# Lynx-MR/orbslam3lib

Measured on AMD Instinct MI355X. Metric: Mfeatures/s extract + Mmatches/s BFMatch, 640x480 stereo 8-level pyr, 1/2/4/8 GPU, higher is better.
Workload: dtype u8; 1 GPU; C2 640x480 stereo, 8 levels x1.2, 2000 feat/frame, FAST 20/7, + per-pair 2000x2000 Hamming kNN2 (left->right, all rows); parallelism=frames sharded across 1 GPU(s), replicas

## Files before the change

### include/orbgpu.h

```cpp
#ifndef ORBGPU_H_
#define ORBGPU_H_

#include <stddef.h>
#include <stdint.h>

#ifdef __cplusplus
extern "C" {
#endif

#define ORBGPU_ABI_VERSION 2

enum {
    ORBGPU_OK = 0,
    ORBGPU_ERR_EMPTY_IMAGE = -1,
    ORBGPU_ERR_CAPACITY = -2,
    ORBGPU_ERR_INVALID = -3,
    ORBGPU_ERR_HIP = -4,
    ORBGPU_ERR_OVERFLOW = -5,
    ORBGPU_ERR_NO_DEVICE = -6,
    ORBGPU_ERR_RUNTIME = -7
};

typedef struct {
    int32_t nfeatures;
// ... 31 lines not shown

int orbgpu_upload_images(orbgpu_ctx* ctx, const uint8_t* images, int n_images, int width,
                         int height, int stride);
uint8_t* orbgpu_device_input(orbgpu_ctx* ctx);
int orbgpu_upload_images_async(orbgpu_ctx* ctx, const uint8_t* images, int n_images, int width,
                               int height, int stride);
int orbgpu_host_alloc(size_t bytes, void** ptr);
int orbgpu_host_free(void* ptr);
int orbgpu_run_batch(orbgpu_ctx* ctx, int n_images, int width, int height, const int32_t* laps,
                     void* stream);
int orbgpu_download_result(orbgpu_ctx* ctx, int image, orbgpu_keypoint* kps, uint8_t* desc,
                           int cap, int* n, int* n_mono);
int orbgpu_download_counts(orbgpu_ctx* ctx, int n_images, int32_t* n, int32_t* n_mono);
int orbgpu_candidate_counts(orbgpu_ctx* ctx, int n_images, int32_t* counts);
int orbgpu_synchronize(orbgpu_ctx* ctx);

int orbgpu_get_pyramid_level(orbgpu_ctx* ctx, int image, int level, int blurred, uint8_t* dst,
                             int dst_stride, int* width, int* height);

int orbgpu_get_level_keypoints(orbgpu_ctx* ctx, int image, orbgpu_keypoint* kps, uint8_t* desc,
                               int cap, int32_t* counts);

int orbgpu_match_knn2(orbgpu_ctx* ctx, const uint8_t* query, int nq, const uint8_t* train, int nt,
                      int32_t* idx1, int32_t* dist1, int32_t* idx2, int32_t* dist2);
int orbgpu_export_descriptors(orbgpu_ctx* ctx, int image, int row0, uint8_t* device_dst, int cap_rows,
                              int* n_rows, void* stream);
int orbgpu_match_knn2_device(orbgpu_ctx* ctx, const uint8_t* d_query, int nq, const uint8_t* d_train, int nt,
                             int32_t* d_idx1, int32_t* d_dist1, int32_t* d_idx2, int32_t* d_dist2, void* stream);

int orbgpu_ingest_images(orbgpu_ctx* ctx, const uint8_t* device_images, int n_images, int width,
// ... 129 lines not shown
```

### orbslam3lib_amd/__init__.py

```python
from __future__ import annotations

import ctypes as C
import os

import numpy as np

__all__ = ["ORBextractor", "ORBmatcher", "BFMatcher", "BatchExtractor", "KEYPOINT_DTYPE", "MAP_POINT_DTYPE",
           "LAST_POINT_DTYPE", "TRACK_POSE_DTYPE", "OrbGpuError", "load_library", "LIB_PATH"]

HERE = os.path.dirname(os.path.abspath(__file__))
LIB_PATH = os.environ.get("ORBGPU_LIB") or os.path.join(HERE, "liborbgpu.so")

MAP_POINT_DTYPE = np.dtype([("proj_x", "<f4"), ("proj_y", "<f4"), ("proj_xr", "<f4"), ("view_cos", "<f4"),
                            ("depth", "<f4"), ("level", "<i4"), ("flags", "<i4"), ("desc", "u1", (32,)),
                            ("proj_yr", "<f4"), ("view_cos_r", "<f4"), ("level_r", "<i4")])
MP_IN_VIEW, MP_BAD, MP_HAS_OBS, MP_IN_VIEW_R = 1, 2, 4, 8

LAST_POINT_DTYPE = np.dtype([("pos", "<f4", (3,)), ("angle", "<f4"), ("octave", "<i4"), ("flags", "<i4"),
                             ("desc", "u1", (32,))])
TRACK_POSE_DTYPE = np.dtype([("Rcw", "<f4", (9,)), ("tcw", "<f4", (3,)), ("Rlw", "<f4", (9,)), ("tlw", "<f4", (3,))])
LP_VALID = 1
TRACK_RIG_DTYPE = np.dtype([("cam_left", "<f4", (8,)), ("Rrl", "<f4", (9,)), ("trl", "<f4", (3,))])

KEYPOINT_DTYPE = np.dtype([("x", "<f4"), ("y", "<f4"), ("size", "<f4"), ("angle", "<f4"),
# ... 5 lines not shown
    "orbgpu_download_result", "orbgpu_download_counts", "orbgpu_synchronize",
    "orbgpu_get_pyramid_level", "orbgpu_get_level_keypoints", "orbgpu_match_knn2",
    "orbgpu_match_stereo_batch", "orbgpu_download_matches", "orbgpu_descriptor_distance",
    "orbgpu_stereo_matches_batch", "orbgpu_download_stereo", "orbgpu_candidate_counts",
    "orbgpu_image_bounds", "orbgpu_undistort_grid_batch", "orbgpu_download_grid",
    "orbgpu_device_sbs_input", "orbgpu_upload_sbs", "orbgpu_ingest_sbs", "orbgpu_pack_soa",
    "orbgpu_download_soa", "orbgpu_download_matches16", "orbgpu_extract_features",
    "orbgpu_search_by_projection_batch", "orbgpu_search_by_projection_stereo",
    "orbgpu_download_projection_matches", "orbgpu_upload_images_async", "orbgpu_host_alloc",
    "orbgpu_host_free", "orbgpu_export_descriptors", "orbgpu_match_knn2_device",
    "orbgpu_set_profiling", "orbgpu_num_stages", "orbgpu_stage_name", "orbgpu_stage_times",
    "orbgpu_reset_stage_times", "orbgpu_last_error", "orbgpu_abi_version",
    "orbgpu_fisheye_stereo_batch", "orbgpu_download_fisheye", "orbgpu_run_batch_match",
    "orbgpu_diagnostic_knobs", "orbgpu_ingest_images", "orbgpu_export_batch_bytes", "orbgpu_export_batch",
    "orbgpu_get_device", "orbgpu_track_by_projection_batch", "orbgpu_download_track_matches",
    "orbgpu_track_by_projection_stereo",
]

DEVICE_CURRENT = -1


class KB8Rig(C.Structure):
    _fields_ = [("cam_left", C.c_float * 8), ("cam_right", C.c_float * 8), ("precision_left", C.c_float),
                ("precision_right", C.c_float), ("R12", C.c_float * 9), ("t12", C.c_float * 3)]

    @classmethod
    def make(cls, cam_left, cam_right, R12=None, t12=(0.0, 0.0, 0.0), precision_left=1e-6,
             precision_right=1e-6):
        r = cls()
        r.cam_left[:] = [float(v) for v in cam_left]
        r.cam_right[:] = [float(v) for v in cam_right]
# ... 395 lines not shown
                                           C.c_void_p(stream) if stream else None))

    def match_stereo(self, stereo_rows_only=False, stream=None):
        _check(_lib.orbgpu_match_stereo_batch(self.ctx.handle, self.n // 2, int(stereo_rows_only),
                                              C.c_void_p(stream) if stream else None))

    def synchronize(self):
        _check(_lib.orbgpu_synchronize(self.ctx.handle))

    def counts(self):
        n = np.zeros(self.n, np.int32)
        m = np.zeros(self.n, np.int32)
        _check(_lib.orbgpu_download_counts(self.ctx.handle, self.n, _p(n), _p(m)))
        return n, m

    def candidate_counts(self):
        c = np.zeros(self.n, np.int32)
        _check(_lib.orbgpu_candidate_counts(self.ctx.handle, self.n, _p(c)))
        return c

    def result(self, i, cap=65536):
        kps = np.zeros(cap, KEYPOINT_DTYPE)
        desc = np.zeros((cap, 32), np.uint8)
        n, m = C.c_int(0), C.c_int(0)
        _check(_lib.orbgpu_download_result(self.ctx.handle, i, _p(kps), _p(desc), cap, C.byref(n),
                                           C.byref(m)))
        return kps[:n.value], desc[:n.value], m.value

    def matches(self, pair, cap=65536):
        out = [np.zeros(cap, np.int32) for _ in range(4)]
# ... 220 lines not shown
```

### orbslam3lib_amd/csrc/orb_ctx.h

```cpp
#pragma once
#include <hip/hip_runtime.h>

#include <algorithm>
#include <cstring>
#include <mutex>
#include <string>
#include <vector>

#include "../../include/orbgpu.h"
#include "orb_geometry.h"
#include "orb_kernels.h"

namespace orbgpu {

int fail(int code, const std::string& msg);

#define HIP_TRY(expr)                                                                  \
    do {                                                                               \
        hipError_t e_ = (expr);                                                        \
        if (e_ != hipSuccess)                                                          \
            return fail(ORBGPU_ERR_HIP, std::string(#expr) + ": " + hipGetErrorString(e_)); \
    } while (0)

enum Stage { ST_RESIZE, ST_BLUR, ST_FAST48, ST_FAST, ST_FAST_TOP, ST_OCTREE, ST_ORIENT, ST_FINAL, ST_KNN,
// ... 90 lines not shown
    int stereo_pairs = 0;
    int fisheye_pairs = 0;
    hipEvent_t fork = nullptr;
    hipEvent_t ext_done = nullptr;
    DevBuf input2{bufs};
    int in_slot = 0, pending_slot = -1;
    hipStream_t copy = nullptr;
    hipEvent_t slot_ready = nullptr;
    std::vector<hipEvent_t> slot_free;
    std::vector<hipEvent_t> join;
    bool serialize = false;
    struct GraphRec { int key[7]; hipGraphExec_t exec; unsigned long long used; };
    std::vector<GraphRec> graphs;
    unsigned long long graph_tick = 0;
    bool last_fused = false;
    std::vector<int32_t> laps_host;
    bool need_fork = true;
    bool restagger = false;
    std::vector<hipEvent_t> stagger_ev;
    std::vector<orbgpu::Chunk> last_chunks;
    int last_images = 0, last_w = 0, last_h = 0, last_pairs = 0;
    unsigned prof_mask = 0;
    std::vector<orbgpu::Pending> pending;
    std::vector<hipEvent_t> event_pool;
    double stage_ms[orbgpu::ST_COUNT] = {};
    long long stage_n[orbgpu::ST_COUNT] = {};
};

namespace orbgpu {

// ... 116 lines not shown
```

### orbslam3lib_amd/csrc/orb_geometry.h

```cpp
#pragma once
#include <algorithm>
#include <cfloat>
#include <climits>
#include <cmath>
#include <cstdlib>
#include <string>
#include <vector>

#include "../../include/orbgpu.h"
#include "orb_fast_cell.h"
#include "orb_kernels.h"
#include "orb_octree.h"

namespace orbgpu {

inline int round_up(int x, int a) { return (x + a - 1) / a * a; }
inline long long round_up_ll(long long x, long long a) { return (x + a - 1) / a * a; }
inline int cv_round_f(float v) { return (int)std::lrintf(v); }
inline int cv_round_d(double v) { return (int)std::lrint(v); }
inline int cv_floor_f(float v) { return (int)std::floor(v); }
inline short sat_short(float v) {
    int i = cv_round_f(v);
    return (short)std::min(std::max(i, (int)SHRT_MIN), (int)SHRT_MAX);
}
// ... 267 lines not shown
        A.oct_split_min_images = 0;
    } else {
        A.oct_split = layout(0) ? 0 : L;
        A.oct_split_min_images = kOctSmallMinImages;
    }
    A.oct_may_retry = 0;
    for (int l = 0; l < L; ++l) {
        const LevelGeom& G = A.lv[l];
        if (G.oct_cap > lds_nodes || G.ncells > A.oct_nq_off / 4) A.oct_may_retry = 1;
        if (l >= A.oct_split && (G.oct_cap > A.oct2_lds_nodes || G.ncells > A.oct2_nq_off / 4)) A.oct_may_retry = 1;
    }
    A.oct_force_retry = K.oct_generic ? 1 : 0;
    A.oct_pyr_max = K.oct_pyr_max;
    A.oct_rounds = K.oct_rounds ? 1 : 0;
    if (A.oct_force_retry) A.oct_may_retry = 1;
}

inline void fast_records(const GeomKnobs& K, GeomPlan& P) {
    BatchArgs& A = P.A;
    const int L = A.nlevels;
    auto fits = [&](int l, int pitch) { return A.lv[l].wCell + 9 <= pitch && A.lv[l].hCell + 6 <= pitch; };
    int tier[kMaxLevels];
    for (int l = 0; l < L; ++l) {
        const int t = fits(l, kCellPitchTiny) ? 0 : fits(l, kCellPitchSmall) ? 1 : 2;
        tier[l] = std::max(t, K.fast_min_tier);
    }
    A.fast_tab_off = (int)P.rtab.size();
    int tier_end[3] = {0, 0, 0}, nrec = 0;
    for (int t = 0; t < 3; ++t) {
        for (int l = 0; l < L; ++l) {
// ... 78 lines not shown
```

### orbslam3lib_amd/csrc/orb_kernels.h

```cpp
#pragma once
#include <hip/hip_runtime.h>
#include <stddef.h>
#include <stdint.h>

namespace orbgpu {

constexpr int kMaxLevels = 16;
constexpr int kMinBorder = 16;
constexpr int kEdge = 19;

__device__ inline int xcd_remap(int orig, int nwg) {
    const int xcd = orig % 8, q = nwg / 8, r = nwg % 8;
    return (xcd < r ? xcd * (q + 1) : r * (q + 1) + (xcd - r) * q) + orig / 8;
}

struct LevelGeom {
    int w, h, pitch;
    long long img_stride;
    int bpitch;
    long long bimg_stride;
    int nCols, nRows, wCell, hCell, maxBX, maxBY;
    int ncells, cell_cap;
    int cell_first;
    long long cellkey_off;
// ... 50 lines not shown
    int* fast_ovf_cnt;
    int fast_qcap;
    int fast_small, fast_ovf_all;
    unsigned long long* octdbg;
    int oct_lds_nodes;
    int oct_lds_bytes;
    int oct_nq_off;
    int oct_split;
    int oct_split_min_images;
    int oct2_threads;
    int oct2_lds_nodes, oct2_lds_bytes, oct2_nq_off, oct2_lds_keys;
    int oct_may_retry;
    int oct_force_retry;
    int oct_pyr_max;
    int oct_rounds;
    int tail0;
    int tail_lds, tail_buf1, tail_tab, tail_maxq, tail_maxrows;
    int tail_min;
    int fuse_out;
};

struct MatchArgs {
    const uint8_t* desc;
    const int32_t* out_n;
    const int32_t* out_mono;
    int out_cap;
    int stereo_only;
    int32_t* idx1;
    int32_t* dist1;
    int32_t* idx2;
// ... 68 lines not shown
    int32_t* cell_start;
    int32_t* cell_idx;
    int img0;
};

constexpr int kOctLdsNodes = 1024;
constexpr int kOdKpBlock = 8;
constexpr int kOdBlockKps = 3 * kOdKpBlock;

constexpr int kOctLdsKeys = 16384;
constexpr int kFastMergeMaxImages = 4;
template <int CP>
constexpr int kFastSmallList() { return CP == 48 ? 512 : 1280; }
constexpr int kFastOvfBlocks = 32;
constexpr int kOctSmallThreads = 256;
constexpr int kOctSmallMinImages = 32;
constexpr int kOctSmallLds = 51 * 1024;

struct OctCfg {
    int nq_off;
    int lds_nodes;
    int lds_keys;
    int lds_bytes;
};

struct OctLayout {
    long long keys, nq, nodemem, total;
};

__host__ __device__ inline long long oct_align(long long x) { return (x + 255) & ~255LL; }
// ... 176 lines not shown
```

### orbslam3lib_amd/csrc/orb_kernels.hip

```cpp
#include <hip/hip_runtime.h>
#include <stdint.h>

#include <algorithm>
#include <atomic>

#include "orb_kernels.h"
#include "orb_math.h"
#include "orb_fast_cell.h"
#include "orb_octree.h"
#include "orb_pattern_data.h"
#include "orb_policy.h"

namespace orbgpu {

static_assert(sizeof(BatchArgs) <= 4096, "kernel argument block too large");

struct PatternTable {
    int8_t v[1024];
};
constexpr int hexval(char c) { return c <= '9' ? c - '0' : c - 'a' + 10; }
constexpr PatternTable make_pattern() {
    PatternTable t{};
    const char* h = ORBGPU_PATTERN_HEX;
    for (int i = 0; i < 1024; ++i) t.v[i] = (int8_t)(hexval(h[2 * i]) * 16 + hexval(h[2 * i + 1]));
// ... 700 lines not shown
    if (nq == 0) return;
    for (int q = blockIdx.x; q < nq; q += gridDim.x) {
        const int2 e = a.fast_ovf[(long long)a.img0 * a.fast_qcap + q];
        fast_cell_one<CP, kList>(a, e.x, e.y, T, M, list, lut, emask, wcnt, wovf, scratch);
        __syncthreads();
    }
    if (threadIdx.x == 0) {
        const int done = __hip_atomic_fetch_add(cnt + 1, 1, __ATOMIC_RELAXED, __HIP_MEMORY_SCOPE_AGENT);
        if (done == (int)gridDim.x - 1) {
            __hip_atomic_store(cnt, 0, __ATOMIC_RELAXED, __HIP_MEMORY_SCOPE_AGENT);
            __hip_atomic_store(cnt + 1, 0, __ATOMIC_RELAXED, __HIP_MEMORY_SCOPE_AGENT);
        }
    }
}

constexpr int kOctRetry = -7;

template <bool kLdsPath>
__device__ __attribute__((always_inline)) inline void octree_level(const BatchArgs& a, int img, int l,
                                                                   uint8_t* nodemem_lds, int* scratch,
                                                                   OctShared& sh, const OctCfg q) {
    const LevelGeom G = a.lv[l];
    DevPolicy p{scratch};
    const int32_t* cnt = a.cellcnt + (long long)img * a.cellcnt_img_stride + G.cellcnt_off;
    const uint32_t* ck = a.cellkeys + (long long)img * a.cellkeys_img_stride + G.cellkey_off;
    uint8_t* ws = a.octws + (long long)img * a.octws_img_stride + G.oct_off;
    const OctLayout L = oct_layout(G.cand_cap, G.oct_cap);
    uint32_t* keys = reinterpret_cast<uint32_t*>(ws + L.keys);
    void* nm = G.oct_cap <= q.lds_nodes ? (void*)nodemem_lds : (void*)(ws + L.nodemem);
    int32_t* cell_off = reinterpret_cast<int32_t*>(nodemem_lds);
    const bool off_in_lds = G.ncells <= q.nq_off / 4;
    if (!off_in_lds) cell_off = reinterpret_cast<int32_t*>(ws + L.nq);
    auto scan_cells = [&]() {
        int carry = 0;
        for (int base = 0; base < G.ncells; base += blockDim.x) {
            const int i = base + threadIdx.x;
            const int v = i < G.ncells ? cnt[i] : 0;
            int tot;
            const int ex = p.scan_excl(v, &tot);
            if (i < G.ncells) cell_off[i] = carry + ex;
            carry += tot;
        }
        __syncthreads();
        return carry;
    };
    const int n = scan_cells();
    uint32_t* out_keys = a.lvlkey + (long long)img * a.lvlkp_img_stride + G.kp_off;
    unsigned long long* dbg = a.octdbg ? a.octdbg + ((long long)img * kMaxLevels + l) * 8 : nullptr;
    int r = n > G.cand_cap ? -3 : 0;
    const bool nodes_fit = off_in_lds && G.oct_cap <= q.lds_nodes && !a.oct_force_retry;
    const int pyr_off = (int)((max(oct_nodemem_bytes(G.oct_cap), (size_t)(4 * G.ncells)) + 15) & ~(size_t)15);
    const int pyrD = kLdsPath && q.lds_bytes > pyr_off && (long long)G.ncells * G.cell_cap < (1 << 24)
                         ? oct_pyr_depth((size_t)(q.lds_bytes - pyr_off), G.W, G.H, a.oct_pyr_max)
                         : 0;
    uint16_t* xtbl = reinterpret_cast<uint16_t*>(nodemem_lds + pyr_off + oct_pyr_bytes(pyrD, oct_nini(G.W, G.H)));
    if (kLdsPath && r == 0 && !nodes_fit) r = kOctRetry;
    if (kLdsPath && r == 0 && n > q.lds_keys) {
        OctWST<kLdsAS, kGlobalAS, kGlobalAS> w;
        w.keys = (asp<kGlobalAS, uint32_t>)keys;
        w.n = n;
        w.nq = (asp<kGlobalAS, uint16_t>)(ws + L.nq);
        w.m = oct_nodemem_carve<kLdsAS>(nodemem_lds, G.oct_cap);
        w.cap = G.oct_cap;
        w.out_keys = (asp<kGlobalAS, uint32_t>)out_keys;
        w.out_cap = G.kp_cap;
        w.dbg = dbg;
        w.cell_off = (asp<kLdsAS, const int32_t>)cell_off;
        w.cellkeys = (asp<kGlobalAS, const uint32_t>)ck;
        w.ncells = G.ncells;
        w.cell_cap = G.cell_cap;
        w.pyr = (asp<kLdsAS, uint32_t>)(nodemem_lds + pyr_off);
        w.pyrD = pyrD;
        w.rounds = a.oct_rounds;
        w.xcode = (asp<kLdsAS, uint16_t>)xtbl;
        w.ycode = (asp<kLdsAS, uint16_t>)(xtbl + G.W + 1);
        r = octree_distribute(p, w, (asp<kLdsAS, OctShared>)&sh, G.W, G.H, G.N);
        if (r == kOctDeep) {
            __syncthreads();
            scan_cells();
            w.pyrD = 0;
            r = octree_distribute(p, w, (asp<kLdsAS, OctShared>)&sh, G.W, G.H, G.N);
        }
    } else if (kLdsPath && r == 0) {
        OctWST<kLdsAS, kGlobalAS> w;
        w.keys = (asp<kGlobalAS, uint32_t>)keys;
        w.n = n;
        w.nq = (asp<kLdsAS, uint16_t>)(nodemem_lds + q.nq_off);
        w.m = oct_nodemem_carve<kLdsAS>(nodemem_lds, G.oct_cap);
        w.cap = G.oct_cap;
        w.out_keys = (asp<kGlobalAS, uint32_t>)out_keys;
        w.out_cap = G.kp_cap;
        w.dbg = dbg;
        w.cell_off = (asp<kLdsAS, const int32_t>)cell_off;
        w.cellkeys = (asp<kGlobalAS, const uint32_t>)ck;
        w.ncells = G.ncells;
        w.cell_cap = G.cell_cap;
        w.pyr = (asp<kLdsAS, uint32_t>)(nodemem_lds + pyr_off);
        w.pyrD = pyrD;
        w.rounds = a.oct_rounds;
        w.xcode = (asp<kLdsAS, uint16_t>)xtbl;
        w.ycode = (asp<kLdsAS, uint16_t>)(xtbl + G.W + 1);
        r = octree_distribute(p, w, (asp<kLdsAS, OctShared>)&sh, G.W, G.H, G.N);
        if (r == kOctDeep) {
            __syncthreads();
            scan_cells();
            w.pyrD = 0;
            r = octree_distribute(p, w, (asp<kLdsAS, OctShared>)&sh, G.W, G.H, G.N);
        }
    } else if (!kLdsPath && r == 0) {
        OctWST<kGeneric, kGeneric> w;
        w.keys = keys;
        w.n = n;
        w.nq = n <= q.lds_keys && off_in_lds ? reinterpret_cast<uint16_t*>(nodemem_lds + q.nq_off)
                                             : reinterpret_cast<uint16_t*>(ws + L.nq);
        w.m = oct_nodemem_carve<kGeneric>(nm, G.oct_cap);
        w.cap = G.oct_cap;
        w.out_keys = out_keys;
        w.out_cap = G.kp_cap;
        w.dbg = dbg;
        w.cell_off = cell_off;
        w.cellkeys = ck;
        w.ncells = G.ncells;
        w.cell_cap = G.cell_cap;
// ... 4 lines not shown
        else r = octree_distribute(p, w, &sh, G.W, G.H, G.N);
    }
    if (threadIdx.x == 0) {
        a.lvlcnt[img * kMaxLevels + l] = r < 0 ? 0 : r;
        a.status[img * kMaxLevels + l] = r < 0 ? r : 0;
    }
}

template <int NT>
__global__ __launch_bounds__(NT) void k_octree(BatchArgs a, int l0, OctCfg q) {
    extern __shared__ __attribute__((aligned(16))) uint8_t nodemem_lds[];
    __shared__ int scratch[16];
    __shared__ OctShared sh;
    octree_level<true>(a, a.img0 + blockIdx.x, l0 + blockIdx.y, nodemem_lds, scratch, sh, q);
}

__global__ __launch_bounds__(512, 1) void k_octree_retry(BatchArgs a) {
    extern __shared__ __attribute__((aligned(16))) uint8_t nodemem_lds[];
    __shared__ int scratch[16];
    __shared__ OctShared sh;
    for (int s = blockIdx.x; s < a.nimages * a.nlevels; s += gridDim.x) {
        const int img = a.img0 + s / a.nlevels, l = s % a.nlevels;
        if (a.status[img * kMaxLevels + l] != kOctRetry) continue;
        octree_level<false>(a, img, l, nodemem_lds, scratch, sh, OctCfg{a.oct_nq_off, a.oct_lds_nodes, kOctLdsKeys, a.oct_lds_bytes});
        __syncthreads();
    }
}

constexpr int kOdLanes = 32;
constexpr int kOdPairs = 256 / kOdLanes;
static_assert(kOdLanes == 32, "k_orient_desc: one disc row and 8 test pairs per lane");
static_assert(kOdKpBlock == 256 / kOdLanes, "orb_kernels.h kOdKpBlock");

constexpr int kOdPatchR = 18;
constexpr int kOdPatchRows = 2 * kOdPatchR + 1;
constexpr int kOdPatchPitch = 48;
constexpr int kOdPatchChunks = kOdPatchRows * 3;
constexpr int kOdPatchIt = (kOdPatchChunks + kOdLanes - 1) / kOdLanes;

__device__ inline int od_sum(int v) {
// ... 616 lines not shown
        hipLaunchKernelGGL((k_fast_cells<kCellPitchSmall, true>), grid, block, 0, s, a, c0, magic);
        hipLaunchKernelGGL(k_fast_cells_ovf<kCellPitchSmall>, dim3(kFastOvfBlocks), oblock, 0, s, a);
    } else if (tile == kCellPitchTiny) hipLaunchKernelGGL((k_fast_cells<kCellPitchTiny, false>), grid, block, 0, s, a, c0, magic);
    else if (tile == kCellPitchSmall) hipLaunchKernelGGL((k_fast_cells<kCellPitchSmall, false>), grid, block, 0, s, a, c0, magic);
    else hipLaunchKernelGGL((k_fast_cells<kCellMax, false>), grid, block, 0, s, a, c0, magic);
    return hipGetLastError();
}
hipError_t launch_octree(const BatchArgs& a, hipStream_t s) {
    constexpr int kMaxDevices = 64;
    static std::atomic<int> lds_set[kMaxDevices];
    int dev = 0;
    if (hipGetDevice(&dev) != hipSuccess || dev < 0 || dev >= kMaxDevices) dev = kMaxDevices - 1;
    std::atomic<int>& set = lds_set[dev];
    if (a.oct_lds_bytes > 65536 && a.oct_lds_bytes > set.load()) {
        for (const void* f : {reinterpret_cast<const void*>(k_octree<512>),
                              reinterpret_cast<const void*>(k_octree_retry)}) {
            hipError_t e = hipFuncSetAttribute(f, hipFuncAttributeMaxDynamicSharedMemorySize, a.oct_lds_bytes);
            if (e != hipSuccess) return e;
        }
        int cur = set.load();
        while (a.oct_lds_bytes > cur && !set.compare_exchange_weak(cur, a.oct_lds_bytes)) {}
    }
    const int split = a.nimages < a.oct_split_min_images ? a.nlevels : std::min(a.oct_split, a.nlevels);
    if (split > 0)
        hipLaunchKernelGGL(k_octree<512>, dim3(a.nimages, split), dim3(512), a.oct_lds_bytes, s, a, 0,
                           OctCfg{a.oct_nq_off, a.oct_lds_nodes, kOctLdsKeys, a.oct_lds_bytes});
    if (split < a.nlevels) {
        const OctCfg q{a.oct2_nq_off, a.oct2_lds_nodes, a.oct2_lds_keys, a.oct2_lds_bytes};
        if (a.oct2_threads == 128)
            hipLaunchKernelGGL(k_octree<128>, dim3(a.nimages, a.nlevels - split), dim3(128), a.oct2_lds_bytes, s, a,
                               split, q);
        else
            hipLaunchKernelGGL(k_octree<256>, dim3(a.nimages, a.nlevels - split), dim3(256), a.oct2_lds_bytes, s, a,
                               split, q);
    }
    if (a.oct_may_retry)
        hipLaunchKernelGGL(k_octree_retry, dim3(std::min(a.nimages * a.nlevels, 64)), dim3(512),
                           a.oct_lds_bytes, s, a);
    return hipGetLastError();
}
hipError_t launch_orient_desc(const BatchArgs& a, hipStream_t s) {
    const uint32_t d = (uint32_t)a.total_od_blocks;
    const uint32_t magic = d > 1 ? 0xFFFFFFFFu / d + 1u : 0u;
    hipLaunchKernelGGL(k_orient_desc, dim3(a.total_od_blocks, a.nimages), dim3(256), 0, s, a, magic);
    return hipGetLastError();
}
hipError_t launch_finalize(const BatchArgs& a, hipStream_t s) {
    if (a.nimages <= 2) hipLaunchKernelGGL(k_finalize<1024>, dim3(a.nimages), dim3(1024), 0, s, a);
    else if (a.nimages <= kFinWideMaxImages) hipLaunchKernelGGL(k_finalize<512>, dim3(a.nimages), dim3(512), 0, s, a);
    else hipLaunchKernelGGL(k_finalize<256>, dim3(a.nimages), dim3(256), 0, s, a);
    return hipGetLastError();
}
hipError_t launch_knn2_pairs(const MatchArgs& m, int npairs, hipStream_t s) {
// ... 24 lines not shown
```

### orbslam3lib_amd/csrc/orb_octree.h

```cpp
#pragma once
#include <hip/hip_runtime.h>
#include <stdint.h>

#include "orb_addrspace.h"
#include "orb_kernels.h"
#include "orb_introsort.h"

namespace orbgpu {

struct alignas(16) OctNode {
    uint16_t x0, y0, x1, y1;
    int32_t cnt;
    uint32_t path;
};
static_assert(sizeof(OctNode) == 16, "OctNode: 16 bytes");

constexpr int kOctPyrMaxD = 7;
constexpr int kOctDeep = -8;
__host__ __device__ inline int pyr_base(int d, int nIni) { return nIni * (((1 << (2 * d)) - 1) / 3); }
__host__ __device__ inline size_t oct_pyr_bytes(int D, int nIni) { return 8 * (size_t)pyr_base(D + 1, nIni); }
__host__ __device__ inline uint32_t oct_path_code(int d, uint32_t idx) { return ((uint32_t)d << 27) | idx; }
__host__ __device__ inline int oct_path_depth(uint32_t code) { return (int)(code >> 27); }
__host__ __device__ inline uint32_t oct_path_idx(uint32_t code) { return code & 0x7FFFFFFu; }
__host__ __device__ inline int oct_nini(int W, int H) {
    const int nIni = (int)roundf((float)W / (float)H);
    return nIni < 1 ? 1 : nIni;
}
__host__ __device__ inline size_t oct_tbl_bytes(int W, int H) { return ((size_t)2 * (W + H + 2) + 15) & ~(size_t)15; }
__host__ __device__ inline int oct_pyr_depth(size_t bytes, int W, int H, int Dmax) {
    const int nIni = oct_nini(W, H);
    const size_t t = oct_tbl_bytes(W, H);
    int D = 0;
    while (D < Dmax && D < kOctPyrMaxD && oct_pyr_bytes(D + 1, nIni) + t <= bytes &&
// ... 150 lines not shown
    n.y1 = (uint16_t)(v.y >> 16);
    n.cnt = (int32_t)v.z;
    n.path = v.w;
    return n;
}
template <class NP>
__host__ __device__ inline void on_st(NP a, int i, OctNode n) {
    orb_u32x4 v;
    v.x = (uint32_t)n.x0 | ((uint32_t)n.y0 << 16);
    v.y = (uint32_t)n.x1 | ((uint32_t)n.y1 << 16);
    v.z = (uint32_t)n.cnt;
    v.w = n.path;
    as_vec4(a)[i] = v;
}

template <int LAS, int GAS, int NAS, class P>
__host__ __device__ __attribute__((always_inline)) inline int octree_distribute(P& p, const OctWST<LAS, GAS, NAS> ws,
                                          asp<LAS, OctShared> sh, int W, int H, int N) {
    const int tid = p.tid(), NT = p.nthreads();
    const int n = ws.n;
    const OctNodeMemT<LAS> M = ws.m;
    auto cur = M.nodesA;
    auto nxt = M.nodesB;
    auto ccur = M.cntA;
    auto cnxt = M.cntB;
    auto vsz = M.vsizeA;
    auto vsz2 = M.vsizeB;
    auto nq = ws.nq;
    const bool nw = p.node_worker();
    unsigned long long t_prev = p.now();
    auto mark = [&](int slot) __attribute__((always_inline)) {
        if (ws.dbg && tid == 0) {
            const unsigned long long t = p.now();
            ws.dbg[slot] += t - t_prev;
            t_prev = t;
        }
    };
    if (ws.cap > 16383) return -3;
    const int nIni = oct_nini(W, H);
    const float hX = (float)W / (float)nIni;
    if (nIni + 4 > ws.cap) return -3;
    const int D = ws.pyrD;
    const bool fast = D > 0;
    auto pcnt = ws.pyr;
    auto pbest = fast ? ws.pyr + pyr_base(D + 1, nIni) : ws.pyr;
    const int bD = pyr_base(D, nIni);
    const bool direct = fast && !ws.rounds;
    if (fast) {
        for (int e = tid; e < (nIni << (2 * D)); e += NT) {
            pcnt[bD + e] = 0;
            pbest[bD + e] = 0;
        }
        for (int e = tid; e <= kOctPyrMaxD; e += NT) sh->tot[e] = 0;
    }
    auto for_keys = [&](auto f) __attribute__((always_inline)) {
        if (n <= 0) return;
        uint32_t key[kOctUnroll], nkey[kOctUnroll];
#pragma unroll
        for (int u = 0; u < kOctUnroll; ++u) {
            const int k = u * NT + tid;
            key[u] = ws.keys[k < n ? k : n - 1];
        }
// ... 151 lines not shown
            prev = size;
            size = (int)(uint32_t)es + frozen;
            X = (int)(uint32_t)es - (int)(es >> 32);
            if (size > ws.cap - 4) {
                status = -3;
                break;
            }
            if (size >= N || size == prev) break;
            final_phase = size + 3 * X > N;
            if (X > 0 && R >= D) {
                status = kOctDeep;
                break;
            }
            if (final_phase) break;
        }
        if (status) return status;
        const int nwork = R > 0 ? (nIni << (2 * (R - 1))) + pyr_base(R - 1, nIni) + nIni : nIni;
        const int bR1 = pyr_base(R + 1, nIni);
        int carry = 0, ccarry = 0;
        for (int base = 0; base < nwork; base += NT) {
            int t = base + tid, d = R;
            const bool in = t < nwork;
            if (in)
                for (; d > 0; --d) {
                    const int w = nIni << (2 * (d - 1));
                    if (t < w) break;
                    t -= w;
                }
            const bool head = d == R;
            uint32_t pp = 0;
            int c[4] = {0, 0, 0, 0};
// ... 135 lines not shown
        ss.lpos = M.undivpos;
        ss.rpos = M.blockoff;
        ss.rank = M.expoff;
        auto seg = reinterpret_cast<asp<LAS, uint16_t>>(M.divrank);
        const int S = C / 16 + 4;
        for (int b = 0; b < 2; ++b) {
            ss.segF[b] = seg + (3 * b + 0) * S;
            ss.segL[b] = seg + (3 * b + 1) * S;
            ss.segD[b] = seg + (3 * b + 2) * S;
        }
        ss.segK = reinterpret_cast<asp<LAS, int32_t>>(seg + 6 * S + 2);
        return ss;
    };
    while (!sh->done) {
        if (++guard > 4096) return -4;
        if (sh->phase != 1) {
            const int m = sh->nexp;
            auto sb = reinterpret_cast<asp<LAS, SortElem>>(nxt);
            for (int j = tid; j < m; j += NT) {
                const int v = vsz[j];
                SortElem e;
                e.size = cur[v].cnt;
                e.ulx = cur[v].x0;
                e.node = v;
                e.pad = 0;
                se_st(sb, j, e);
            }
            p.sync();
            introsort_partition<LAS>(p, sb, m, sort_scratch(cnxt), &sh->jstop);
        }
        if (sh->phase != 1) {
            p.sync();
            introsort_final<LAS>(p, reinterpret_cast<asp<LAS, SortElem>>(nxt), sh->nexp,
                                 sort_scratch(cnxt));
            p.sync();
            mark(3);
        }
        if (nw) {
            auto np = p.node();
            const int ntid = np.tid(), NNT = np.nthreads();
            const int size = sh->size;
            const int phase = sh->phase;
            if (ntid == 0) sh->prev_size = size;
            if (phase == 1) {
                int carry = 0;
                for (int base = 0; base < size; base += NNT) {
                    const int i = base + ntid;
                    const int v = (i < size && cur[i].cnt > 1) ? 1 : 0;
                    int tot;
                    const int ex = np.scan_small(v, &tot);
                    if (i < size) M.divrank[i] = v ? carry + ex : -1;
                    carry += tot;
                }
                if (ntid == 0) sh->ndiv = carry;
                int c1 = 0, c2 = 0;
                for (int base = 0; base < size; base += NNT) {
                    const int i = base + ntid;
// ... 124 lines not shown
                            if (ccur[4 * i + q] > 1) vsz2[e++] = M.childpos[4 * i + q];
                    }
                    carry += tot;
                }
                if (ntid == 0) sh->nundiv = carry;
            }
            np.sync();
            if (ntid == 0) {
                const int nsize = sh->nchild + sh->nundiv;
                sh->size = nsize;
                if (nsize > ws.cap - 4) {
                    sh->status = -3;
                    sh->done = 1;
                } else if (nsize >= N || nsize == sh->prev_size) {
                    sh->done = 1;
                } else if (sh->phase == 1 && nsize + sh->nexp * 3 > N) {
                    sh->phase = 2;
                }
                if (!sh->done && sh->deep) {
                    sh->status = kOctDeep;
                    sh->done = 1;
                }
                if (ws.dbg) ws.dbg[7] += phase == 1 ? (1ull << 32) + 1ull : 1ull;
            }
            mark(4);
        }
        p.sync();
        mark(2);
        if (fast && !sh->done) {
            const int ne = sh->nexp;
            for (int j = tid; j < ne; j += NT) {
                const int pos = vsz2[j];
                const uint32_t path = nxt[pos].path;
                const int b = pyr_base(oct_path_depth(path) + 1, nIni) + 4 * (int)oct_path_idx(path);
                for (int qq = 0; qq < 4; ++qq) cnxt[4 * pos + qq] = (int)pcnt[b + qq];
            }
        }
        if (!fast) for_keys([&](int base, const uint32_t* key) __attribute__((always_inline)) {
// ... 26 lines not shown
        });
        {
            auto t = cur;
            cur = nxt;
            nxt = t;
            auto c = ccur;
            ccur = cnxt;
            cnxt = c;
            auto u = vsz;
            vsz = vsz2;
            vsz2 = u;
        }
        p.sync();
        mark(fast ? 2 : 5);
    }
    if (sh->status) return sh->status;

    const int size = sh->size;
    if (size > ws.out_cap) return -5;
    if (fast) {
        for (int i = tid; i < size; i += NT) {
            const uint32_t path = cur[i].path;
            const uint32_t v = pbest[pyr_base(oct_path_depth(path), nIni) + (int)oct_path_idx(path)];
            const int kid = (int)(0xFFFFFFu - (v & 0xFFFFFFu));
            ws.out_keys[i] = ws.cell_off ? ws.cellkeys[kid] : ws.keys[kid];
        }
        p.sync();
        mark(2);
        return size;
    }
    auto best = reinterpret_cast<asp<LAS, uint32_t>>(cnxt);
// ... 28 lines not shown
```

### orbslam3lib_amd/csrc/orb_runtime.cpp

```cpp
#include <link.h>

#include <cstdio>
#include <cstdlib>

#include "orb_ctx.h"

using namespace orbgpu;

namespace {

thread_local std::string g_err;

constexpr size_t kGraphCacheSize = 4;

inline int kChunksFor(int n) { return n >= 256 ? 2 : 3; }

bool diagnostics_on() {
    const char* g = getenv("ORBGPU_DIAGNOSTICS");
    return g && std::strcmp(g, "1") == 0;
}

struct KnobDef {
    const char* name;
    void (*parse)(DiagKnobs& k, const char* v);
// ... 462 lines not shown
    if (slot_switch)
        for (const Chunk& ch : chunks) HIP_TRY(hipStreamWaitEvent(ch.st, c->slot_ready, 0));
    const bool stagger = (relayout || c->restagger) && c->knobs.stagger && chunks.size() > 1 && !c->serialize;
    if (stagger) c->restagger = false;
    while (stagger && c->stagger_ev.size() < chunks.size()) {
        hipEvent_t ev;
        HIP_TRY(hipEventCreateWithFlags(&ev, hipEventDisableTiming));
        c->stagger_ev.push_back(ev);
    }
    auto chunk_args = [&](const Chunk& ch) {
        BatchArgs B = A;
        B.img0 = ch.img0;
        B.nimages = ch.n;
        return B;
    };
    auto each = [&](int stage, auto launch) -> int {
        if (isolates(c, chunks, stage))
            return isolated(c, chunks, [&](hipStream_t s0) {
                return timed(c, stage, s0, [&] { return launch(A, s0); });
            });
        for (const Chunk& ch : chunks) {
            const BatchArgs B = chunk_args(ch);
            if (int rr = timed(c, stage, ch.st, [&] { return launch(B, ch.st); })) return rr;
        }
        return 0;
    };
    auto launch_all = [&]() -> int {
        int r = 0;
        int chunk_images = 0;
        for (const Chunk& ch : chunks) chunk_images = std::max(chunk_images, ch.n);
// ... 129 lines not shown

int orbgpu_run_batch(orbgpu_ctx* c, int n, int w, int h, const int32_t* laps, void* stream) {
    return run_batch_impl(c, n, w, h, laps, stream, 0, 0, nullptr);
}

int orbgpu_run_batch_match(orbgpu_ctx* c, int n, int w, int h, const int32_t* laps, int stereo_rows_only,
                           void* stream) {
    if (!c) return fail(ORBGPU_ERR_INVALID, "null ctx");
    if (n < 2 || (n % 2) != 0) return fail(ORBGPU_ERR_INVALID, "run_batch_match needs whole stereo pairs");
    bool matched = false;
    int r = run_batch_impl(c, n, w, h, laps, stream, n / 2, stereo_rows_only ? 1 : 0, &matched);
    if (r || matched) return r;
    return orbgpu_match_stereo_batch(c, n / 2, stereo_rows_only, stream);
}

int orbgpu_synchronize(orbgpu_ctx* c) {
    if (!c) return fail(ORBGPU_ERR_INVALID, "null ctx");
    if (int e_ = ctx_sync(c, true)) return e_;
    resolve_pending(c);
    if (c->knobs.oct_stamps && c->octdbg.p && c->last_images > 0) {
        const int n = c->last_images, L = c->prm.nlevels;
        std::vector<unsigned long long> d((size_t)n * kMaxLevels * 8);
        D2H(d.data(), c->octdbg.p, d.size() * 8);
        for (int l = 0; l < L; ++l) {
            double acc[8] = {}, phase1 = 0;
            for (int i = 0; i < n; ++i) {
                const unsigned long long* s = &d[((size_t)i * kMaxLevels + l) * 8];
                for (int k = 0; k < 7; ++k) acc[k] += (double)s[k];
                acc[7] += (double)(s[7] & 0xFFFFFFFFull);
                phase1 += (double)(s[7] >> 32);
// ... 164 lines not shown
```

Measured before the change: 585.5 Mfeatures/s.

## Add lean octree kernel specialization with compact retry fallback

Adds a compile-time 'lean' instantiation of the octree distribution kernel, used when the host proves every level fits in LDS with a usable pyramid. It strips the debug timing, the phase-1 rounds logic, the deep-rerun path and the global cell-offset fallback. Cases the lean kernel cannot handle return a retry status, and a smaller retry kernel (32 blocks of 128 threads) picks them up, scanning status in strides to skip empty work. The aim is lower register and instruction overhead in the hot octree kernel. The cost is an extra retry launch on every lean batch and more code paths to keep consistent.

```diff
diff --git a/include/orbgpu.h b/include/orbgpu.h
--- a/include/orbgpu.h
+++ b/include/orbgpu.h
@@ -69,6 +69,7 @@
 int orbgpu_download_counts(orbgpu_ctx* ctx, int n_images, int32_t* n, int32_t* n_mono);
 int orbgpu_candidate_counts(orbgpu_ctx* ctx, int n_images, int32_t* counts);
 int orbgpu_synchronize(orbgpu_ctx* ctx);
+int orbgpu_octree_lean(const orbgpu_ctx* ctx);
 
 int orbgpu_get_pyramid_level(orbgpu_ctx* ctx, int image, int level, int blurred, uint8_t* dst,
                              int dst_stride, int* width, int* height);
diff --git a/orbslam3lib_amd/__init__.py b/orbslam3lib_amd/__init__.py
--- a/orbslam3lib_amd/__init__.py
+++ b/orbslam3lib_amd/__init__.py
@@ -43,7 +43,7 @@
     "orbgpu_fisheye_stereo_batch", "orbgpu_download_fisheye", "orbgpu_run_batch_match",
     "orbgpu_diagnostic_knobs", "orbgpu_ingest_images", "orbgpu_export_batch_bytes", "orbgpu_export_batch",
     "orbgpu_get_device", "orbgpu_track_by_projection_batch", "orbgpu_download_track_matches",
-    "orbgpu_track_by_projection_stereo",
+    "orbgpu_track_by_projection_stereo", "orbgpu_octree_lean",
 ]
 
 DEVICE_CURRENT = -1
@@ -469,6 +469,9 @@
         _check(_lib.orbgpu_download_counts(self.ctx.handle, self.n, _p(n), _p(m)))
         return n, m
 
+    def octree_lean(self):
+        return bool(_check(_lib.orbgpu_octree_lean(self.ctx.handle)))
+
     def candidate_counts(self):
         c = np.zeros(self.n, np.int32)
         _check(_lib.orbgpu_candidate_counts(self.ctx.handle, self.n, _p(c)))
diff --git a/orbslam3lib_amd/csrc/orb_ctx.h b/orbslam3lib_amd/csrc/orb_ctx.h
--- a/orbslam3lib_amd/csrc/orb_ctx.h
+++ b/orbslam3lib_amd/csrc/orb_ctx.h
@@ -128,6 +128,7 @@
     std::vector<GraphRec> graphs;
     unsigned long long graph_tick = 0;
     bool last_fused = false;
+    bool last_oct_lean = false;
     std::vector<int32_t> laps_host;
     bool need_fork = true;
     bool restagger = false;
diff --git a/orbslam3lib_amd/csrc/orb_geometry.h b/orbslam3lib_amd/csrc/orb_geometry.h
--- a/orbslam3lib_amd/csrc/orb_geometry.h
+++ b/orbslam3lib_amd/csrc/orb_geometry.h
@@ -305,6 +305,30 @@
     A.oct_pyr_max = K.oct_pyr_max;
     A.oct_rounds = K.oct_rounds ? 1 : 0;
     if (A.oct_force_retry) A.oct_may_retry = 1;
+    A.oct_no_lean = K.oct_rounds || K.oct_generic || K.oct_pyr_max == 0 || K.oct_small_lds != kOctSmallLds ||
+                    K.oct_small_threads != kOctSmallThreads;
+}
+
+inline int octree_split(const BatchArgs& A, int nimages) {
+    return nimages < A.oct_split_min_images ? A.nlevels : std::min(A.oct_split, A.nlevels);
+}
+
+inline bool octree_lean_ok(const BatchArgs& A, int nimages) {
+    if (A.oct_no_lean || A.oct_force_retry || A.oct_rounds || A.oct_pyr_max <= 0 || A.octdbg) return false;
+    const int split = octree_split(A, nimages);
+    for (int l = 0; l < A.nlevels; ++l) {
+        const LevelGeom& G = A.lv[l];
+        const bool small = l >= split;
+        const int nq_off = small ? A.oct2_nq_off : A.oct_nq_off;
+        const int nodes = small ? A.oct2_lds_nodes : A.oct_lds_nodes;
+        const int bytes = small ? A.oct2_lds_bytes : A.oct_lds_bytes;
+        if (G.oct_cap > nodes || G.ncells > nq_off / 4) return false;
+        const long long pyr_off =
+            (long long)((std::max(oct_nodemem_bytes(G.oct_cap), (size_t)(4 * G.ncells)) + 15) & ~(size_t)15);
+        if (bytes <= pyr_off || (long long)G.ncells * G.cell_cap >= (1 << 24)) return false;
+        if (oct_pyr_depth((size_t)(bytes - pyr_off), G.W, G.H, A.oct_pyr_max) < 1) return false;
+    }
+    return true;
 }
 
 inline void fast_records(const GeomKnobs& K, GeomPlan& P) {
diff --git a/orbslam3lib_amd/csrc/orb_kernels.h b/orbslam3lib_amd/csrc/orb_kernels.h
--- a/orbslam3lib_amd/csrc/orb_kernels.h
+++ b/orbslam3lib_amd/csrc/orb_kernels.h
@@ -88,6 +88,7 @@
     int oct_force_retry;
     int oct_pyr_max;
     int oct_rounds;
+    int oct_no_lean;
     int tail0;
     int tail_lds, tail_buf1, tail_tab, tail_maxq, tail_maxrows;
     int tail_min;
@@ -186,6 +187,7 @@
 constexpr int kFastSmallList() { return CP == 48 ? 512 : 1280; }
 constexpr int kFastOvfBlocks = 32;
 constexpr int kOctSmallThreads = 256;
+constexpr int kOctLeanRetryGrid = 32, kOctLeanRetryThreads = 128;
 constexpr int kOctSmallMinImages = 32;
 constexpr int kOctSmallLds = 51 * 1024;
 
diff --git a/orbslam3lib_amd/csrc/orb_kernels.hip b/orbslam3lib_amd/csrc/orb_kernels.hip
--- a/orbslam3lib_amd/csrc/orb_kernels.hip
+++ b/orbslam3lib_amd/csrc/orb_kernels.hip
@@ -7,6 +7,7 @@
 #include "orb_kernels.h"
 #include "orb_math.h"
 #include "orb_fast_cell.h"
+#include "orb_geometry.h"
 #include "orb_octree.h"
 #include "orb_pattern_data.h"
 #include "orb_policy.h"
@@ -738,12 +739,11 @@
     }
 }
 
-constexpr int kOctRetry = -7;
-
-template <bool kLdsPath>
+template <bool kLdsPath, bool kLean = false>
 __device__ __attribute__((always_inline)) inline void octree_level(const BatchArgs& a, int img, int l,
                                                                    uint8_t* nodemem_lds, int* scratch,
                                                                    OctShared& sh, const OctCfg q) {
+    static_assert(kLdsPath || !kLean, "the lean instantiation is an LDS one");
     const LevelGeom G = a.lv[l];
     DevPolicy p{scratch};
     const int32_t* cnt = a.cellcnt + (long long)img * a.cellcnt_img_stride + G.cellcnt_off;
@@ -754,9 +754,10 @@
     void* nm = G.oct_cap <= q.lds_nodes ? (void*)nodemem_lds : (void*)(ws + L.nodemem);
     int32_t* cell_off = reinterpret_cast<int32_t*>(nodemem_lds);
     const bool off_in_lds = G.ncells <= q.nq_off / 4;
-    if (!off_in_lds) cell_off = reinterpret_cast<int32_t*>(ws + L.nq);
+    if (!kLean && !off_in_lds) cell_off = reinterpret_cast<int32_t*>(ws + L.nq);
     auto scan_cells = [&]() {
         int carry = 0;
+        if (kLean && !off_in_lds) return 0;
         for (int base = 0; base < G.ncells; base += blockDim.x) {
             const int i = base + threadIdx.x;
             const int v = i < G.ncells ? cnt[i] : 0;
@@ -770,7 +771,7 @@
     };
     const int n = scan_cells();
     uint32_t* out_keys = a.lvlkey + (long long)img * a.lvlkp_img_stride + G.kp_off;
-    unsigned long long* dbg = a.octdbg ? a.octdbg + ((long long)img * kMaxLevels + l) * 8 : nullptr;
+    unsigned long long* dbg = !kLean && a.octdbg ? a.octdbg + ((long long)img * kMaxLevels + l) * 8 : nullptr;
     int r = n > G.cand_cap ? -3 : 0;
     const bool nodes_fit = off_in_lds && G.oct_cap <= q.lds_nodes && !a.oct_force_retry;
     const int pyr_off = (int)((max(oct_nodemem_bytes(G.oct_cap), (size_t)(4 * G.ncells)) + 15) & ~(size_t)15);
@@ -778,12 +779,9 @@
                          ? oct_pyr_depth((size_t)(q.lds_bytes - pyr_off), G.W, G.H, a.oct_pyr_max)
                          : 0;
     uint16_t* xtbl = reinterpret_cast<uint16_t*>(nodemem_lds + pyr_off + oct_pyr_bytes(pyrD, oct_nini(G.W, G.H)));
-    if (kLdsPath && r == 0 && !nodes_fit) r = kOctRetry;
-    if (kLdsPath && r == 0 && n > q.lds_keys) {
-        OctWST<kLdsAS, kGlobalAS, kGlobalAS> w;
+    auto lds_ws = [&](auto& w) {
         w.keys = (asp<kGlobalAS, uint32_t>)keys;
         w.n = n;
-        w.nq = (asp<kGlobalAS, uint16_t>)(ws + L.nq);
         w.m = oct_nodemem_carve<kLdsAS>(nodemem_lds, G.oct_cap);
         w.cap = G.oct_cap;
         w.out_keys = (asp<kGlobalAS, uint32_t>)out_keys;
@@ -795,42 +793,36 @@
         w.cell_cap = G.cell_cap;
         w.pyr = (asp<kLdsAS, uint32_t>)(nodemem_lds + pyr_off);
         w.pyrD = pyrD;
-        w.rounds = a.oct_rounds;
+        w.rounds = kLean ? 0 : a.oct_rounds;
         w.xcode = (asp<kLdsAS, uint16_t>)xtbl;
         w.ycode = (asp<kLdsAS, uint16_t>)(xtbl + G.W + 1);
-        r = octree_distribute(p, w, (asp<kLdsAS, OctShared>)&sh, G.W, G.H, G.N);
-        if (r == kOctDeep) {
+    };
+    auto with_rerun = [&](auto& w) {
+        int rr = octree_distribute(p, w, (asp<kLdsAS, OctShared>)&sh, G.W, G.H, G.N);
+        if (rr == kOctDeep) {
             __syncthreads();
             scan_cells();
             w.pyrD = 0;
-            r = octree_distribute(p, w, (asp<kLdsAS, OctShared>)&sh, G.W, G.H, G.N);
-        }
+            rr = octree_distribute(p, w, (asp<kLdsAS, OctShared>)&sh, G.W, G.H, G.N);
+        }
+        return rr;
+    };
+    if (kLdsPath && r == 0 && !nodes_fit) r = kOctRetry;
+    if (kLean && r == 0) {
+        OctWST<kLdsAS, kGlobalAS> w;
+        lds_ws(w);
+        w.nq = nullptr;
+        r = octree_distribute<true>(p, w, (asp<kLdsAS, OctShared>)&sh, G.W, G.H, G.N);
+    } else if (kLdsPath && r == 0 && n > q.lds_keys) {
+        OctWST<kLdsAS, kGlobalAS, kGlobalAS> w;
+        lds_ws(w);
+        w.nq = (asp<kGlobalAS, uint16_t>)(ws + L.nq);
+        r = with_rerun(w);
     } else if (kLdsPath && r == 0) {
         OctWST<kLdsAS, kGlobalAS> w;
-        w.keys = (asp<kGlobalAS, uint32_t>)keys;
-        w.n = n;
+        lds_ws(w);
         w.nq = (asp<kLdsAS, uint16_t>)(nodemem_lds + q.nq_off);
-        w.m = oct_nodemem_carve<kLdsAS>(nodemem_lds, G.oct_cap);
-        w.cap = G.oct_cap;
-        w.out_keys = (asp<kGlobalAS, uint32_t>)out_keys;
-        w.out_cap = G.kp_cap;
-        w.dbg = dbg;
-        w.cell_off = (asp<kLdsAS, const int32_t>)cell_off;
-        w.cellkeys = (asp<kGlobalAS, const uint32_t>)ck;
-        w.ncells = G.ncells;
-        w.cell_cap = G.cell_cap;
-        w.pyr = (asp<kLdsAS, uint32_t>)(nodemem_lds + pyr_off);
-        w.pyrD = pyrD;
-        w.rounds = a.oct_rounds;
-        w.xcode = (asp<kLdsAS, uint16_t>)xtbl;
-        w.ycode = (asp<kLdsAS, uint16_t>)(xtbl + G.W + 1);
-        r = octree_distribute(p, w, (asp<kLdsAS, OctShared>)&sh, G.W, G.H, G.N);
-        if (r == kOctDeep) {
-            __syncthreads();
-            scan_cells();
-            w.pyrD = 0;
-            r = octree_distribute(p, w, (asp<kLdsAS, OctShared>)&sh, G.W, G.H, G.N);
-        }
+        r = with_rerun(w);
     } else if (!kLdsPath && r == 0) {
         OctWST<kGeneric, kGeneric> w;
         w.keys = keys;
@@ -865,16 +857,30 @@
     __shared__ OctShared sh;
     octree_level<true>(a, a.img0 + blockIdx.x, l0 + blockIdx.y, nodemem_lds, scratch, sh, q);
 }
-
-__global__ __launch_bounds__(512, 1) void k_octree_retry(BatchArgs a) {
+template <int NT>
+__global__ __launch_bounds__(NT) void k_octree_lean(BatchArgs a, int l0, OctCfg q) {
     extern __shared__ __attribute__((aligned(16))) uint8_t nodemem_lds[];
     __shared__ int scratch[16];
     __shared__ OctShared sh;
-    for (int s = blockIdx.x; s < a.nimages * a.nlevels; s += gridDim.x) {
-        const int img = a.img0 + s / a.nlevels, l = s % a.nlevels;
-        if (a.status[img * kMaxLevels + l] != kOctRetry) continue;
-        octree_level<false>(a, img, l, nodemem_lds, scratch, sh, OctCfg{a.oct_nq_off, a.oct_lds_nodes, kOctLdsKeys, a.oct_lds_bytes});
-        __syncthreads();
+    octree_level<true, true>(a, a.img0 + blockIdx.x, l0 + blockIdx.y, nodemem_lds, scratch, sh, q);
+}
+
+__global__ __launch_bounds__(512, 1) void k_octree_retry(BatchArgs a, OctCfg q0, OctCfg q1, int split) {
+    extern __shared__ __attribute__((aligned(16))) uint8_t nodemem_lds[];
+    __shared__ int scratch[16];
+    __shared__ OctShared sh;
+    const int total = a.nimages * a.nlevels, G = (int)gridDim.x, NT = (int)blockDim.x;
+    auto is_retry = [&](int s) {
+        return s < total && a.status[(a.img0 + s / a.nlevels) * kMaxLevels + s % a.nlevels] == kOctRetry;
+    };
+    for (int base = blockIdx.x; base < total; base += NT * G) {
+        if (!__syncthreads_or(is_retry(base + (int)threadIdx.x * G))) continue;
+        for (int s = base; s < total && s < base + NT * G; s += G) {
+            if (!is_retry(s)) continue;
+            const int l = s % a.nlevels;
+            octree_level<false>(a, a.img0 + s / a.nlevels, l, nodemem_lds, scratch, sh, l < split ? q0 : q1);
+            __syncthreads();
+        }
     }
 }
 
@@ -1521,6 +1527,7 @@
     std::atomic<int>& set = lds_set[dev];
     if (a.oct_lds_bytes > 65536 && a.oct_lds_bytes > set.load()) {
         for (const void* f : {reinterpret_cast<const void*>(k_octree<512>),
+                              reinterpret_cast<const void*>(k_octree_lean<512>),
                               reinterpret_cast<const void*>(k_octree_retry)}) {
             hipError_t e = hipFuncSetAttribute(f, hipFuncAttributeMaxDynamicSharedMemorySize, a.oct_lds_bytes);
             if (e != hipSuccess) return e;
@@ -1528,22 +1535,35 @@
         int cur = set.load();
         while (a.oct_lds_bytes > cur && !set.compare_exchange_weak(cur, a.oct_lds_bytes)) {}
     }
-    const int split = a.nimages < a.oct_split_min_images ? a.nlevels : std::min(a.oct_split, a.nlevels);
-    if (split > 0)
-        hipLaunchKernelGGL(k_octree<512>, dim3(a.nimages, split), dim3(512), a.oct_lds_bytes, s, a, 0,
-                           OctCfg{a.oct_nq_off, a.oct_lds_nodes, kOctLdsKeys, a.oct_lds_bytes});
+    const int split = geom::octree_split(a, a.nimages);
+    const bool lean = geom::octree_lean_ok(a, a.nimages);
+    if (split > 0) {
+        const OctCfg q{a.oct_nq_off, a.oct_lds_nodes, kOctLdsKeys, a.oct_lds_bytes};
+        if (lean) hipLaunchKernelGGL(k_octree_lean<512>, dim3(a.nimages, split), dim3(512), a.oct_lds_bytes, s, a, 0, q);
+        else hipLaunchKernelGGL(k_octree<512>, dim3(a.nimages, split), dim3(512), a.oct_lds_bytes, s, a, 0, q);
+    }
     if (split < a.nlevels) {
         const OctCfg q{a.oct2_nq_off, a.oct2_lds_nodes, a.oct2_lds_keys, a.oct2_lds_bytes};
-        if (a.oct2_threads == 128)
+        if (lean)
+            hipLaunchKernelGGL(k_octree_lean<kOctSmallThreads>, dim3(a.nimages, a.nlevels - split),
+                               dim3(kOctSmallThreads), a.oct2_lds_bytes, s, a, split, q);
+        else if (a.oct2_threads == 128)
             hipLaunchKernelGGL(k_octree<128>, dim3(a.nimages, a.nlevels - split), dim3(128), a.oct2_lds_bytes, s, a,
                                split, q);
         else
             hipLaunchKernelGGL(k_octree<256>, dim3(a.nimages, a.nlevels - split), dim3(256), a.oct2_lds_bytes, s, a,
                                split, q);
     }
-    if (a.oct_may_retry)
-        hipLaunchKernelGGL(k_octree_retry, dim3(std::min(a.nimages * a.nlevels, 64)), dim3(512),
-                           a.oct_lds_bytes, s, a);
+    const OctCfg qr{a.oct_nq_off, a.oct_lds_nodes, kOctLdsKeys, a.oct_lds_bytes};
+    if (a.oct_may_retry) {
+        hipLaunchKernelGGL(k_octree_retry, dim3(std::min(a.nimages * a.nlevels, 64)), dim3(512), a.oct_lds_bytes, s, a,
+                           qr, qr, 0);
+    } else if (lean) {
+        const OctCfg q2{a.oct2_nq_off, a.oct2_lds_nodes, a.oct2_lds_keys, a.oct2_lds_bytes};
+        const int lds = std::max(split > 0 ? a.oct_lds_bytes : 0, split < a.nlevels ? a.oct2_lds_bytes : 0);
+        hipLaunchKernelGGL(k_octree_retry, dim3(std::min(a.nimages * a.nlevels, kOctLeanRetryGrid)),
+                           dim3(kOctLeanRetryThreads), lds, s, a, qr, q2, split);
+    }
     return hipGetLastError();
 }
 hipError_t launch_orient_desc(const BatchArgs& a, hipStream_t s) {
diff --git a/orbslam3lib_amd/csrc/orb_octree.h b/orbslam3lib_amd/csrc/orb_octree.h
--- a/orbslam3lib_amd/csrc/orb_octree.h
+++ b/orbslam3lib_amd/csrc/orb_octree.h
@@ -17,6 +17,7 @@
 
 constexpr int kOctPyrMaxD = 7;
 constexpr int kOctDeep = -8;
+constexpr int kOctRetry = -7;
 __host__ __device__ inline int pyr_base(int d, int nIni) { return nIni * (((1 << (2 * d)) - 1) / 3); }
 __host__ __device__ inline size_t oct_pyr_bytes(int D, int nIni) { return 8 * (size_t)pyr_base(D + 1, nIni); }
 __host__ __device__ inline uint32_t oct_path_code(int d, uint32_t idx) { return ((uint32_t)d << 27) | idx; }
@@ -197,7 +198,7 @@
     as_vec4(a)[i] = v;
 }
 
-template <int LAS, int GAS, int NAS, class P>
+template <bool kLean = false, int LAS, int GAS, int NAS, class P>
 __host__ __device__ __attribute__((always_inline)) inline int octree_distribute(P& p, const OctWST<LAS, GAS, NAS> ws,
                                           asp<LAS, OctShared> sh, int W, int H, int N) {
     const int tid = p.tid(), NT = p.nthreads();
@@ -211,9 +212,9 @@
     auto vsz2 = M.vsizeB;
     auto nq = ws.nq;
     const bool nw = p.node_worker();
-    unsigned long long t_prev = p.now();
+    unsigned long long t_prev = kLean ? 0ull : p.now();
     auto mark = [&](int slot) __attribute__((always_inline)) {
-        if (ws.dbg && tid == 0) {
+        if (!kLean && ws.dbg && tid == 0) {
             const unsigned long long t = p.now();
             ws.dbg[slot] += t - t_prev;
             t_prev = t;
@@ -224,11 +225,12 @@
     const float hX = (float)W / (float)nIni;
     if (nIni + 4 > ws.cap) return -3;
     const int D = ws.pyrD;
-    const bool fast = D > 0;
+    if (kLean && D <= 0) return kOctRetry;
+    const bool fast = kLean || D > 0;
     auto pcnt = ws.pyr;
     auto pbest = fast ? ws.pyr + pyr_base(D + 1, nIni) : ws.pyr;
     const int bD = pyr_base(D, nIni);
-    const bool direct = fast && !ws.rounds;
+    const bool direct = kLean || (fast && !ws.rounds);
     if (fast) {
         for (int e = tid; e < (nIni << (2 * D)); e += NT) {
             pcnt[bD + e] = 0;
@@ -410,7 +412,7 @@
             }
             if (final_phase) break;
         }
-        if (status) return status;
+        if (status) return kLean && status == kOctDeep ? kOctRetry : status;
         const int nwork = R > 0 ? (nIni << (2 * (R - 1))) + pyr_base(R - 1, nIni) + nIni : nIni;
         const int bR1 = pyr_base(R + 1, nIni);
         int carry = 0, ccarry = 0;
@@ -576,7 +578,8 @@
     };
     while (!sh->done) {
         if (++guard > 4096) return -4;
-        if (sh->phase != 1) {
+        const bool final_round = kLean || sh->phase != 1;
+        if (final_round) {
             const int m = sh->nexp;
             auto sb = reinterpret_cast<asp<LAS, SortElem>>(nxt);
             for (int j = tid; j < m; j += NT) {
@@ -591,7 +594,7 @@
             p.sync();
             introsort_partition<LAS>(p, sb, m, sort_scratch(cnxt), &sh->jstop);
         }
-        if (sh->phase != 1) {
+        if (final_round) {
             p.sync();
             introsort_final<LAS>(p, reinterpret_cast<asp<LAS, SortElem>>(nxt), sh->nexp,
                                  sort_scratch(cnxt));
@@ -602,7 +605,7 @@
             auto np = p.node();
             const int ntid = np.tid(), NNT = np.nthreads();
             const int size = sh->size;
-            const int phase = sh->phase;
+            const int phase = kLean ? 2 : sh->phase;
             if (ntid == 0) sh->prev_size = size;
             if (phase == 1) {
                 int carry = 0;
@@ -757,14 +760,14 @@
                     sh->done = 1;
                 } else if (nsize >= N || nsize == sh->prev_size) {
                     sh->done = 1;
-                } else if (sh->phase == 1 && nsize + sh->nexp * 3 > N) {
+                } else if (!kLean && sh->phase == 1 && nsize + sh->nexp * 3 > N) {
                     sh->phase = 2;
                 }
                 if (!sh->done && sh->deep) {
                     sh->status = kOctDeep;
                     sh->done = 1;
                 }
-                if (ws.dbg) ws.dbg[7] += phase == 1 ? (1ull << 32) + 1ull : 1ull;
+                if (!kLean && ws.dbg) ws.dbg[7] += phase == 1 ? (1ull << 32) + 1ull : 1ull;
             }
             mark(4);
         }
@@ -821,7 +824,7 @@
         p.sync();
         mark(fast ? 2 : 5);
     }
-    if (sh->status) return sh->status;
+    if (sh->status) return kLean && sh->status == kOctDeep ? kOctRetry : sh->status;
 
     const int size = sh->size;
     if (size > ws.out_cap) return -5;
diff --git a/orbslam3lib_amd/csrc/orb_runtime.cpp b/orbslam3lib_amd/csrc/orb_runtime.cpp
--- a/orbslam3lib_amd/csrc/orb_runtime.cpp
+++ b/orbslam3lib_amd/csrc/orb_runtime.cpp
@@ -500,6 +500,12 @@
         B.nimages = ch.n;
         return B;
     };
+    if (isolates(c, chunks, ST_OCTREE)) {
+        c->last_oct_lean = geom::octree_lean_ok(A, A.nimages);
+    } else {
+        c->last_oct_lean = true;
+        for (const Chunk& ch : chunks) c->last_oct_lean = c->last_oct_lean && geom::octree_lean_ok(chunk_args(ch), ch.n);
+    }
     auto each = [&](int stage, auto launch) -> int {
         if (isolates(c, chunks, stage))
             return isolated(c, chunks, [&](hipStream_t s0) {
@@ -659,6 +665,12 @@
     return orbgpu_match_stereo_batch(c, n / 2, stereo_rows_only, stream);
 }
 
+int orbgpu_octree_lean(const orbgpu_ctx* c) {
+    if (!c) return fail(ORBGPU_ERR_INVALID, "null ctx");
+    if (c->last_images <= 0) return fail(ORBGPU_ERR_INVALID, "no batch has run");
+    return c->last_oct_lean ? 1 : 0;
+}
+
 int orbgpu_synchronize(orbgpu_ctx* c) {
     if (!c) return fail(ORBGPU_ERR_INVALID, "null ctx");
     if (int e_ = ctx_sync(c, true)) return e_;
```

After: 585.0 Mfeatures/s. About the same (-0.1%).
